# ucsdmanorlab/PSSR2

Hardware: AMD Instinct MI355X
Metric: HR tiles/sec (512^2 4xSR) train (higher is better)
Workload: dtype bf16

## Files before the change

include/pssr_mi355.h:

```cpp
#ifndef PSSR_MI355_H
#define PSSR_MI355_H

#include <stdint.h>

#ifdef __cplusplus
extern "C" {
#endif

typedef void* pssr_stream_t;

enum { PSSR_F32 = 0, PSSR_BF16 = 1, PSSR_F16 = 2 };

enum {
    PSSR_OK = 0,
    PSSR_ERR_ARG = -1,
    PSSR_ERR_LAUNCH = -2,
    PSSR_ERR_UNSUPPORTED = -3
};

int pssr_abi_version(void);
const char* pssr_last_error(void);

int pssr_pack_conv_weight(const float* w_oihw, void* packed, int cout, int cin, int ks,
                          int ci_begin, int ci_count, int mode, const int32_t* n_perm,
// ... 140 lines not shown
int pssr_f64_to_f32(const double* in, float* out, int n, int accumulate, int stripes, pssr_stream_t stream);

int pssr_ssim_level_fwd(const float* x, const float* y, int planes, int h, int w, const float* win_host,
                        int k, float c1, float c2, double* sums, double* l1_sum, pssr_stream_t stream);
int pssr_avgpool2_planes(const float* in, float* out, int planes, int h, int w, pssr_stream_t stream);
int pssr_msssim_weights(const double* sums, int levels, int planes, const double* nvalid,
                        const float* level_weights, int ms, float mix, const double* l1_sum,
                        double l1_numel, const float* grad_out, float* loss_out, float* wts,
                        float* l1_coef, pssr_stream_t stream);
int pssr_ssim_level_bwd(const float* x, const float* y, int planes, int h, int w, const float* win_host,
                        int k, float c1, float c2, const float* wts, int use_ssim, const float* dcoarse,
                        int hc, int wc, const float* l1_coef, float* dx, pssr_stream_t stream);

int pssr_ssim_level_fwd_adj(const float* x, const float* y, float in_div, int planes, int h, int w, const float* win_host, int k,
                            float c1, float c2, int use_ssim, double* sums, double* l1_sum, int stripes, int64_t stripe_stride,
                            float* adj, pssr_stream_t stream);
int pssr_msssim_weights_striped(const double* sums, int stripes, int64_t stripe_stride, double* folded, int levels, int planes,
                                const double* nvalid, const float* level_weights, int ms, float mix, const double* l1_sum,
                                double l1_numel, const float* grad_out, float* loss_out, float* wts, float* l1_coef,
                                pssr_stream_t stream);
int pssr_ssim_level_bwd_adj(const float* x, const float* y, float in_div, const float* adj, int planes, int h, int w,
                            const float* win_host, int k, const float* wts, const float* dcoarse, int hc, int wc,
                            const float* l1_coef, float* dx, pssr_stream_t stream);
int pssr_avgpool2_planes_div(const float* in, float in_div, float* out, int planes, int h, int w, pssr_stream_t stream);
int pssr_avgpool2_pair_div(const float* x, const float* y, float in_div, float* xo, float* yo, int planes, int h, int w,
                           pssr_stream_t stream);

int pssr_adamw_step(float* p, const float* g, float* m, float* v, int64_t n, float lr, float beta1,
                    float beta2, float eps, float weight_decay, int64_t step, float grad_scale,
                    pssr_stream_t stream);
int pssr_adamw_step_dev(float* p, const float* g, float* m, float* v, int64_t n, int64_t* state,
                        float beta1, float beta2, float eps, float weight_decay, float grad_scale,
                        pssr_stream_t stream);
int pssr_amp_check(const float* g, int64_t n, int32_t* amp, pssr_stream_t stream);
int pssr_adamw_step_amp(float* p, const float* g, float* m, float* v, int64_t n, int64_t* state,
                        float beta1, float beta2, float eps, float weight_decay, float grad_scale,
                        int32_t* amp, float growth, float backoff, int interval, pssr_stream_t stream);

int pssr_bilinear_down_u8(const uint8_t* hr, uint8_t* tmp, uint8_t* lr, int planes, int H, int W,
                          int h, int w, pssr_stream_t stream);
int pssr_u8_to_f32(const uint8_t* in, float* out, int64_t n, pssr_stream_t stream);
int pssr_crappify_gaussian(const float* in, float* out, int tiles, int64_t per_tile, float intensity,
                           float gain, float spread, uint64_t seed, uint64_t tile_offset,
                           const double* noise, int flags, const uint64_t* tile_counter,
                           pssr_stream_t stream);
int pssr_crappify_poisson(const float* in, float* out, int tiles, int64_t per_tile, float intensity,
// ... 152 lines not shown
```

pssr2_amd/_lib.py:

```python
from __future__ import annotations

import ctypes as C
import os
from pathlib import Path

_LIB_PATH = Path(__file__).resolve().parent / "libpssr_mi355.so"
_lib = None

F32, BF16, F16 = 0, 1, 2
PRO_NONE, PRO_BN_RELU, PRO_GELU = 0, 1, 2
EPI_STORE, EPI_TAIL, EPI_DGRAD_MASK, EPI_FINAL, EPI_DGRAD_GELU, EPI_HEADQ = 0, 1, 2, 3, 4, 5
FLAG_RELU, FLAG_STATS, FLAG_AFFINE, FLAG_HEADQ, FLAG_SHUF2, FLAG_SOLO = 1, 2, 4, 8, 16, 32

c_void_p, c_int, c_i64, c_float = C.c_void_p, C.c_int, C.c_int64, C.c_float


class ConvDesc(C.Structure):
    _fields_ = [
        ("dtype", C.c_int32), ("n", C.c_int32), ("h", C.c_int32), ("w", C.c_int32),
        ("in0", c_void_p), ("in0_cstride", C.c_int32), ("in0_coff", C.c_int32), ("cin0", C.c_int32), ("taps0", C.c_int32),
        ("w0", c_void_p),
        ("in1", c_void_p), ("in1_cstride", C.c_int32), ("in1_coff", C.c_int32), ("cin1", C.c_int32), ("taps1", C.c_int32),
        ("w1", c_void_p),
        ("prologue", C.c_int32), ("pro_scale", c_void_p), ("pro_shift", c_void_p),
        ("out", c_void_p), ("out_cstride", C.c_int32), ("out_coff", C.c_int32), ("cout", C.c_int32), ("n_pad", C.c_int32),
        ("bias", c_void_p),
        ("epilogue", C.c_int32), ("flags", C.c_int32),
        ("aux", c_void_p), ("aux_cstride", C.c_int32), ("aux_coff", C.c_int32),
        ("aux_scale", c_void_p), ("aux_shift", c_void_p), ("aux_mean", c_void_p), ("aux_invstd", c_void_p),
        ("stats", c_void_p),
# ... 33 lines not shown
    _fields_ = [("w", C.c_void_p * DWPACK_BATCH_MAX), ("packed", C.c_void_p * DWPACK_BATCH_MAX), ("c", C.c_int32 * DWPACK_BATCH_MAX),
                ("flip", C.c_int32 * DWPACK_BATCH_MAX)]


class CopyBatch(C.Structure):
    _fields_ = [("dst", C.c_void_p * COPY_BATCH_MAX), ("src", C.c_void_p * COPY_BATCH_MAX), ("n", C.c_int64 * COPY_BATCH_MAX)]


class PackItem(C.Structure):
    _fields_ = [("w", c_void_p), ("packed", c_void_p), ("n_perm", c_void_p),
                ("cout", C.c_int32), ("cin", C.c_int32), ("ks", C.c_int32), ("ci_begin", C.c_int32), ("ci_count", C.c_int32),
                ("mode", C.c_int32), ("k_pad", C.c_int32), ("n_pad", C.c_int32), ("dtype", C.c_int32), ("center", C.c_int32)]


def lib():
    global _lib
    if _lib is None:
        if not _LIB_PATH.exists():
            raise RuntimeError(
                f"{_LIB_PATH} not found: build the HIP extension first (python -c 'import __graft_entry__ as g; g.build()' "
                "or make -C pssr2_amd/csrc). pssr2_amd has no CPU fallback.")
        import torch
        _lib = C.CDLL(str(_LIB_PATH))
        _lib.pssr_last_error.restype = C.c_char_p
        _lib.pssr_packed_weight_bytes.restype = C.c_int64
        _lib.pssr_conv2d_workspace_bytes.restype = C.c_int64
        _lib.pssr_gradhist_workspace_bytes.restype = C.c_int64
    return _lib


def check(status: int, what: str):
    if status != 0:
        raise RuntimeError(f"{what} failed ({status}): {lib().pssr_last_error().decode()}")


def ptr(t):
    return None if t is None else c_void_p(t.data_ptr())


def stream_ptr():
    import torch
    return c_void_p(torch.cuda.current_stream().cuda_stream)
```

pssr2_amd/csrc/api_common.cpp:

```cpp
#include <stdarg.h>
#include <stdio.h>
#include <stdlib.h>
#include <string.h>

#include <mutex>

#include "tunables.h"

static thread_local char g_err[512] = "";

void pssr_set_error(const char* fmt, ...) {
    va_list ap;
    va_start(ap, fmt);
    vsnprintf(g_err, sizeof(g_err), fmt, ap);
    va_end(ap);
}

extern "C" const char* pssr_last_error(void) { return g_err; }
extern "C" int pssr_abi_version(void) { return 4; }

namespace {
struct Entry { const char* name; int PssrTunables::*field; int dflt; int lo, hi; };
const Entry kEntries[] = {
    {"IGEMM_FLAT", &PssrTunables::igemm_flat, 1, 0, 1},
    {"IGEMM_BIG", &PssrTunables::igemm_big, 1, 0, 2},
    {"IGEMM_V3", &PssrTunables::igemm_v3, 1, 0, 2},
    {"IGEMM_V3_64", &PssrTunables::igemm_v3_64, 1, 0, 1},
    {"V3_LDS_PAD", &PssrTunables::v3_lds_pad, 0, 0, 100},
    {"IGEMM_DBG", &PssrTunables::igemm_dbg, 0, 0, 255},
    {"IGEMM_N64", &PssrTunables::igemm_n64, 1, 0, 1},
    {"IGEMM_KSPLIT", &PssrTunables::igemm_ksplit, 384, 1, 1 << 20},
    {"CONV_EPI8", &PssrTunables::conv_epi8, 1, 0, 1},
    {"WGRAD_LEAN", &PssrTunables::wgrad_lean, 1, 0, 1},
    {"WGRAD_X2", &PssrTunables::wgrad_x2, 0, 0, 1},
    {"WGRAD_DMA", &PssrTunables::wgrad_dma, 1, 0, 1},
    {"WGRAD_BLOCKS", &PssrTunables::wgrad_blocks, 256, 1, 1 << 20},
    {"WGRAD_BLOCKS_1X1", &PssrTunables::wgrad_blocks_1x1, 384, 1, 1 << 20},
    {"DWCONV_TILE", &PssrTunables::dwconv_tile, 1, 0, 1},
    {"DWWG_BLOCKS", &PssrTunables::dwwg_blocks, 1024, 1, 1 << 20},
    {"LN_BWD_BLOCKS", &PssrTunables::ln_bwd_blocks, 256, 1, 1 << 20},
    {"LN_DBG", &PssrTunables::ln_dbg, 0, 0, 3},
};
PssrTunables g_tun;
std::once_flag g_tun_once;
void tun_init() {
    for (const Entry& e : kEntries) {
        char key[64];
        snprintf(key, sizeof(key), "PSSR_%s", e.name);
        const char* v = getenv(key);
        int x = v ? atoi(v) : e.dflt;
        if (x < e.lo || x > e.hi) x = e.dflt;
        g_tun.*(e.field) = x;
    }
}
}

PssrTunables& pssr_tunables() {
    std::call_once(g_tun_once, tun_init);
    return g_tun;
}

extern "C" int pssr_set_option(const char* name, int value) {
    if (name == nullptr) { pssr_set_error("pssr_set_option: null name"); return PSSR_ERR_ARG; }
    PssrTunables& t = pssr_tunables();
// ... 20 lines not shown
```

pssr2_amd/csrc/loss.hip:

```cpp
#include "common.h"

namespace {

constexpr int TS = 32;
constexpr int MAXW = 33;

struct Win { float g[MAXW]; int k; };

template <int K_DUMMY>
__global__ __launch_bounds__(256) void ssim_fwd_kernel(const float* __restrict__ X, const float* __restrict__ Y, int H, int W,
                                                       Win win, float C1, float C2, double* sums ,
                                                       double* l1_sum ) {
    extern __shared__ float lds[];
    const int k = win.k, halo = k - 1, IN = TS + halo;
    float* xs = lds;
    float* ys = xs + IN * IN;
    float* hp = ys + IN * IN;
    const int plane = blockIdx.z;
    const int oy0 = blockIdx.y * TS, ox0 = blockIdx.x * TS;
    const int VH = H - halo, VW = W - halo;
    const float* xp = X + (long)plane * H * W;
    const float* yp = Y + (long)plane * H * W;
    const int tid = threadIdx.x;
    float l1 = 0.f;
// ... 353 lines not shown
            const float cs = (2.f * sxy + C2) / Dcs;
            const float Dl = mx * mx + my * my + C1;
            const float lum = (2.f * mx * my + C1) / Dl;
            cs_acc += cs; ss_acc += lum * cs;
        }
    }
    __shared__ float red[3][256];
    red[0][tid] = cs_acc; red[1][tid] = ss_acc; red[2][tid] = l1;
    __syncthreads();
    for (int o = 128; o > 0; o >>= 1) {
        if (tid < o) { red[0][tid] += red[0][tid + o]; red[1][tid] += red[1][tid + o]; red[2][tid] += red[2][tid + o]; }
        __syncthreads();
    }
    if (tid == 0) {
        atomicAdd(sums + plane * 2, (double)red[0][0]);
        atomicAdd(sums + plane * 2 + 1, (double)red[1][0]);
        if (l1_sum) atomicAdd(l1_sum, (double)red[2][0]);
    }
}

template <int K>
__global__ __launch_bounds__(256) void ssim_fwd_adj_k(const float* __restrict__ X, const float* __restrict__ Y, int H, int W,
                                                      Win win, float C1, float C2, double* sums, double* l1_sum, int stripes, long stripe_stride,
                                                      float* __restrict__ adj, int use_ssim, float in_mul) {
    constexpr int halo = K - 1, IN = TS + halo, SEG = 8, NS = TS / SEG;
    constexpr int HPW = TS + 1;
    extern __shared__ float lds[];
    float* xs = lds;
    float* ys = xs + IN * IN;
    float* hp = ys + IN * IN;
    const int plane = blockIdx.z;
    const int oy0 = blockIdx.y * TS, ox0 = blockIdx.x * TS;
    const int VH = H - halo, VW = W - halo;
    const float* xp = X + (long)plane * H * W;
    const float* yp = Y + (long)plane * H * W;
    const int tid = threadIdx.x;
    float l1 = 0.f;
    for (int i = tid; i < IN * IN; i += 256) {
        const int r = i / IN, c = i % IN;
        const int gy = oy0 + r, gx = ox0 + c;
        float xv = 0.f, yv = 0.f;
        if (gy < H && gx < W) { xv = __fmul_rn(xp[(long)gy * W + gx], in_mul); yv = __fmul_rn(yp[(long)gy * W + gx], in_mul); }
        xs[i] = xv; ys[i] = yv;
    }
    __syncthreads();
    if (l1_sum) {
        constexpr int r5 = K / 2;
        float wsum = 0.f;
#pragma unroll
        for (int t = 0; t < K; ++t) wsum += win.g[t];
        for (int i = tid; i < TS * TS; i += 256) {
            const int r = i / TS, c = i % TS;
            const int gy = oy0 + r, gx = ox0 + c;
            if (gy < H && gx < W) {
                float sy = wsum, sx = wsum;
                if (gy < r5 || gy >= H - r5) {
                    sy = 0.f;
#pragma unroll
                    for (int t = 0; t < K; ++t) { const int yy = gy + t - r5; if (yy >= 0 && yy < H) sy += win.g[t]; }
                }
                if (gx < r5 || gx >= W - r5) {
                    sx = 0.f;
#pragma unroll
                    for (int t = 0; t < K; ++t) { const int xx = gx + t - r5; if (xx >= 0 && xx < W) sx += win.g[t]; }
                }
                l1 += fabsf(xs[r * IN + c] - ys[r * IN + c]) * sy * sx;
            }
        }
// ... 46 lines not shown
            if (use_ssim) {
                const float dl_dmx = 2.f * (my - lum * mx) / Dl;
                a = lum * dcs_dmx + cs * dl_dmx; b = lum * dcs_dexx; cc = lum * dcs_dexy;
            }
            float* ap = adj + ((long)plane * 3 * H + (oy0 + vr0 + j)) * W + ox0 + vc;
            ap[0] = a; ap[(long)H * W] = b; ap[2L * H * W] = cc;
        }
    }
    __shared__ float red[3][256];
    red[0][tid] = cs_acc; red[1][tid] = ss_acc; red[2][tid] = l1;
    __syncthreads();
    for (int o = 128; o > 0; o >>= 1) {
        if (tid < o) { red[0][tid] += red[0][tid + o]; red[1][tid] += red[1][tid + o]; red[2][tid] += red[2][tid + o]; }
        __syncthreads();
    }
    if (tid == 0) {
        const long so = (long)((blockIdx.x + blockIdx.y * 5) % stripes) * stripe_stride, lo = (long)stripes * stripe_stride;
        stat_add(sums + so + plane * 2, lo, red[0][0]);
        stat_add(sums + so + plane * 2 + 1, lo, red[1][0]);
        if (l1_sum) stat_add(l1_sum + so, lo, red[2][0]);
    }
}

template <int K>
__global__ __launch_bounds__(256) void ssim_bwd_adj_k(const float* __restrict__ X, const float* __restrict__ Y, const float* __restrict__ ADJ,
                                                      int H, int W, Win win, const float* __restrict__ wts,
                                                      const float* __restrict__ dcoarse, int HC, int WC, const float* l1_coef_p,
                                                      float* __restrict__ dX, float in_mul) {
    constexpr int halo = K - 1, AD = TS + halo;
    constexpr int SEG = 8, NS = TS / SEG;
    constexpr int ADC = AD + 1;
    constexpr int THR = AD + SEG, THW = TS + 1;
    constexpr int NL = (AD * AD + 255) / 256;
    extern __shared__ float lds[];
    float* ad = lds;
    float* th = lds + AD * ADC;
    const int plane = blockIdx.z;
    const int qy0 = blockIdx.y * TS, qx0 = blockIdx.x * TS;
    const int VH = H - halo, VW = W - halo;
    const float* xp = X + (long)plane * H * W;
    const float* yp = Y + (long)plane * H * W;
    const float* ap = ADJ + (long)plane * 3 * H * W;
    const int tid = threadIdx.x;
    const float wt = wts[plane];
    int goff[NL], lslot[NL];
#pragma unroll
    for (int u = 0; u < NL; ++u) {
        const int i = tid + u * 256;
        const int r = i / AD, c = i - r * AD;
        const int py = qy0 - halo + r, px = qx0 - halo + c;
        lslot[u] = i < AD * AD ? r * ADC + c : -1;
        goff[u] = (i < AD * AD && py >= 0 && py < VH && px >= 0 && px < VW) ? py * W + px : -1;
    }
    float pre[NL];
#define SB_LOAD(Q)                                                                                                \
    _Pragma("unroll") for (int u = 0; u < NL; ++u) pre[u] = goff[u] >= 0 ? wt * ap[(long)(Q) * H * W + goff[u]] : 0.f;
    SB_LOAD(0)
    const bool vitem = tid < TS * NS;
    const int vc = tid % TS, vr0 = (tid / TS) * SEG;
    float xv[SEG], yv[SEG], gsum[SEG];
#pragma unroll
    for (int o = 0; o < SEG; ++o) {
        const int gy = qy0 + vr0 + o, gx = qx0 + vc;
        const bool ok = vitem && gy < H && gx < W;
        xv[o] = ok ? __fmul_rn(xp[(long)gy * W + gx], in_mul) : 0.f;
        yv[o] = ok ? __fmul_rn(yp[(long)gy * W + gx], in_mul) : 0.f;
        gsum[o] = 0.f;
    }
#pragma unroll
    for (int q = 0; q < 3; ++q) {
#pragma unroll
        for (int u = 0; u < NL; ++u) if (lslot[u] >= 0) ad[lslot[u]] = pre[u];
        __syncthreads();
        if (q < 2) { SB_LOAD(q + 1) }
        for (int it = tid; it < AD * NS; it += 256) {
            const int r = it / NS, c0 = (it % NS) * SEG;
            float v[SEG + K - 1];
#pragma unroll
            for (int j = 0; j < SEG + K - 1; ++j) v[j] = ad[r * ADC + c0 + j];
#pragma unroll
            for (int o = 0; o < SEG; ++o) {
                float s_ = 0.f;
#pragma unroll
                for (int t = 0; t < K; ++t) s_ = fmaf(win.g[t], v[o + halo - t], s_);
                th[r * THW + c0 + o] = s_;
            }
        }
        __syncthreads();
        if (vitem) {
            float v[SEG + K - 1];
#pragma unroll
            for (int j = 0; j < SEG + K - 1; ++j) v[j] = th[(vr0 + j) * THW + vc];
#pragma unroll
            for (int o = 0; o < SEG; ++o) {
                float a = 0.f;
#pragma unroll
                for (int t = 0; t < K; ++t) a = fmaf(win.g[t], v[o + halo - t], a);
                if (q == 0) gsum[o] = a;
                else if (q == 1) gsum[o] = gsum[o] + 2.f * xv[o] * a;
                else gsum[o] = gsum[o] + yv[o] * a;
            }
        }
    }
#undef SB_LOAD
    if (!vitem) return;
    const float l1c = l1_coef_p ? l1_coef_p[0] : 0.f;
    constexpr int r5 = K / 2;
    float wsum = 0.f;
#pragma unroll
    for (int t = 0; t < K; ++t) wsum += win.g[t];
    float* dxp = dX + (long)plane * H * W;
#pragma unroll
    for (int o = 0; o < SEG; ++o) {
        const int gy = qy0 + vr0 + o, gx = qx0 + vc;
        if (gy >= H || gx >= W) continue;
        float g = gsum[o];
        if (dcoarse) {
            const int cy = (gy + (H & 1)) >> 1, cx = (gx + (W & 1)) >> 1;
            g += 0.25f * dcoarse[((long)plane * HC + cy) * WC + cx];
        }
        if (l1c != 0.f) {
            float sy = wsum, sx = wsum;
            if (gy < r5 || gy >= H - r5) {
                sy = 0.f;
#pragma unroll
                for (int t = 0; t < K; ++t) { const int yy = gy + t - r5; if (yy >= 0 && yy < H) sy += win.g[t]; }
            }
            if (gx < r5 || gx >= W - r5) {
                sx = 0.f;
#pragma unroll
                for (int t = 0; t < K; ++t) { const int xx = gx + t - r5; if (xx >= 0 && xx < W) sx += win.g[t]; }
            }
            const float d = xv[o] - yv[o];
            g += l1c * sy * sx * (d > 0.f ? 1.f : (d < 0.f ? -1.f : 0.f));
        }
        dxp[(long)gy * W + gx] = __fmul_rn(g, in_mul);
// ... 173 lines not shown
int pssr_ssim_level_fwd(const float* x, const float* y, int planes, int h, int w, const float* win_host, int k,
                        float c1, float c2, double* sums, double* l1_sum, pssr_stream_t s) {
    PSSR_CHECK(x && y && sums && win_host && planes > 0 && k > 0 && k <= MAXW && (k & 1), PSSR_ERR_ARG, "ssim_level_fwd: bad args");
    PSSR_CHECK(h >= k && w >= k, PSSR_ERR_ARG, "ssim_level_fwd: image %dx%d smaller than window %d", h, w, k);
    const int IN = TS + k - 1;
    const size_t lds = (size_t)(2 * IN * IN + 5 * IN * (TS + 1)) * sizeof(float);
    const int eh = l1_sum ? h : h - k + 1, ew = l1_sum ? w : w - k + 1;
    static bool attr = false;
    if (!attr) {
        (void)hipFuncSetAttribute((const void*)ssim_fwd_kernel<0>, hipFuncAttributeMaxDynamicSharedMemorySize, 160 * 1024 - 4096);
        (void)hipFuncSetAttribute((const void*)ssim_fwd_k<11>, hipFuncAttributeMaxDynamicSharedMemorySize, 160 * 1024 - 4096);
        attr = true;
    }
    if (k == 11)
        hipLaunchKernelGGL(ssim_fwd_k<11>, dim3(cdiv(ew, TS), cdiv(eh, TS), planes), dim3(256), lds, (hipStream_t)s, x, y, h, w,
                           make_win(win_host, k), c1, c2, sums, l1_sum);
    else
        hipLaunchKernelGGL(ssim_fwd_kernel<0>, dim3(cdiv(ew, TS), cdiv(eh, TS), planes), dim3(256), lds, (hipStream_t)s, x, y, h, w,
                           make_win(win_host, k), c1, c2, sums, l1_sum);
    PSSR_LAUNCH_CHECK();
    return PSSR_OK;
}

int pssr_ssim_level_fwd_adj(const float* x, const float* y, float in_div, int planes, int h, int w, const float* win_host, int k, float c1,
                            float c2, int use_ssim, double* sums, double* l1_sum, int stripes, int64_t stripe_stride, float* adj,
                            pssr_stream_t s) {
    PSSR_CHECK(x && y && sums && win_host && planes > 0 && adj && k == 11, PSSR_ERR_ARG,
               "ssim_level_fwd_adj: needs the adjoint buffer and the 11-tap window (k=%d)", k);
    PSSR_CHECK(h >= k && w >= k && stripes >= 1 && (stripes == 1 || stripe_stride > 0) && in_div > 0.f, PSSR_ERR_ARG, "ssim_level_fwd_adj: bad size / stripes / in_div");
    const int IN = TS + k - 1;
    const size_t lds = (size_t)(2 * IN * IN + IN * (TS + 1)) * sizeof(float);
    const int eh = l1_sum ? h : h - k + 1, ew = l1_sum ? w : w - k + 1;
    hipLaunchKernelGGL(ssim_fwd_adj_k<11>, dim3(cdiv(ew, TS), cdiv(eh, TS), planes), dim3(256), lds, (hipStream_t)s, x, y, h, w,
                       make_win(win_host, k), c1, c2, sums, l1_sum, stripes, (long)stripe_stride, adj, use_ssim, in_div == 1.f ? 1.f : 1.f / in_div);
    PSSR_LAUNCH_CHECK();
    return PSSR_OK;
}

int pssr_ssim_level_bwd_adj(const float* x, const float* y, float in_div, const float* adj, int planes, int h, int w, const float* win_host,
                            int k, const float* wts, const float* dcoarse, int hc, int wc, const float* l1_coef, float* dx, pssr_stream_t s) {
    PSSR_CHECK(x && y && adj && wts && dx && win_host && planes > 0 && k == 11, PSSR_ERR_ARG, "ssim_level_bwd_adj: bad args (k=%d)", k);
    constexpr int AD = TS + 10;
    const size_t lds = (size_t)(AD * (AD + 1) + (AD + 8) * (TS + 1)) * sizeof(float);
    hipLaunchKernelGGL(ssim_bwd_adj_k<11>, dim3(cdiv(w, TS), cdiv(h, TS), planes), dim3(256), lds, (hipStream_t)s, x, y, adj, h, w,
                       make_win(win_host, k), wts, dcoarse, hc, wc, l1_coef, dx, in_div == 1.f ? 1.f : 1.f / in_div);
    PSSR_LAUNCH_CHECK();
    return PSSR_OK;
}

int pssr_avgpool2_planes(const float* in, float* out, int planes, int h, int w, pssr_stream_t s) {
    return pssr_avgpool2_planes_div(in, 1.f, out, planes, h, w, s);
}

int pssr_avgpool2_planes_div(const float* in, float in_div, float* out, int planes, int h, int w, pssr_stream_t s) {
    PSSR_CHECK(in && out && planes > 0 && h > 0 && w > 0 && in_div > 0.f, PSSR_ERR_ARG, "avgpool2_planes: bad args");
    const int ho = (h + 2 * (h & 1) - 2) / 2 + 1, wo = (w + 2 * (w & 1) - 2) / 2 + 1;
    const long total = (long)planes * ho * wo;
    int blocks = (int)((total + 255) / 256); if (blocks > 8192) blocks = 8192;
    hipLaunchKernelGGL(avgpool_kernel, dim3(blocks), dim3(256), 0, (hipStream_t)s, in, out, in, out, planes, h, w, ho, wo, in_div == 1.f ? 1.f : 1.f / in_div);
    PSSR_LAUNCH_CHECK();
    return PSSR_OK;
}

int pssr_avgpool2_pair_div(const float* x, const float* y, float in_div, float* xo, float* yo, int planes, int h, int w, pssr_stream_t s) {
    PSSR_CHECK(x && y && xo && yo && planes > 0 && h > 0 && w > 0 && in_div > 0.f, PSSR_ERR_ARG, "avgpool2_pair: bad args");
    const int ho = (h + 2 * (h & 1) - 2) / 2 + 1, wo = (w + 2 * (w & 1) - 2) / 2 + 1;
    const long total = (long)planes * ho * wo;
    int blocks = (int)((total + 255) / 256); if (blocks > 8192) blocks = 8192;
    hipLaunchKernelGGL(avgpool_kernel, dim3(blocks, 2), dim3(256), 0, (hipStream_t)s, x, xo, y, yo, planes, h, w, ho, wo, in_div == 1.f ? 1.f : 1.f / in_div);
    PSSR_LAUNCH_CHECK();
// ... 49 lines not shown
```

pssr2_amd/csrc/tunables.h:

```cpp
#pragma once
#include "../../include/pssr_mi355.h"

struct PssrTunables {
    int igemm_flat;
    int igemm_big;
    int igemm_v3;
    int igemm_v3_64;
    int v3_lds_pad;
    int igemm_dbg;
    int igemm_n64;
    int igemm_ksplit;
    int conv_epi8;
    int wgrad_lean;
    int wgrad_x2;
    int wgrad_dma;
    int wgrad_blocks;
    int wgrad_blocks_1x1;
    int dwconv_tile;
    int dwwg_blocks;
    int ln_bwd_blocks;
    int ln_dbg;
};
PssrTunables& pssr_tunables();
```

pssr2_amd/ops.py:

```python
from __future__ import annotations

import ctypes as C

import torch

from . import _lib as L

TORCH_DTYPE = {L.F32: torch.float32, L.BF16: torch.bfloat16, L.F16: torch.float16}


def dtype_code(dt: torch.dtype) -> int:
    if dt == torch.float32:
        return L.F32
    if dt == torch.bfloat16:
        return L.BF16
    if dt == torch.float16:
        return L.F16
    raise ValueError(f"unsupported compute dtype {dt}; use torch.float32, torch.bfloat16 or torch.float16")


def pad_to(v: int, m: int) -> int:
    return (v + m - 1) // m * m


# ... 210 lines not shown

def f64_to_f32_batch(items, stripes=STAT_STRIPES):
    for k in range(0, len(items), L.COPY_BATCH_MAX):
        chunk = items[k:k + L.COPY_BATCH_MAX]
        fb = L.FoldBatch()
        for i, (src, dst, acc) in enumerate(chunk):
            if src.dtype != torch.float64 or dst.dtype != torch.float32 or src.numel() < stripes * dst.numel() or not (src.is_contiguous() and dst.is_contiguous()):
                raise ValueError("f64_to_f32_batch needs contiguous float64 [stripes * n] sources and float32 [n] destinations")
            fb.dst[i], fb.src[i], fb.n[i], fb.accumulate[i] = dst.data_ptr(), src.data_ptr(), dst.numel(), int(acc)
        L.check(L.lib().pssr_f64_to_f32_batch(C.byref(fb), len(chunk), stripes, L.stream_ptr()), "pssr_f64_to_f32_batch")


def _win(win):
    arr = (C.c_float * len(win))(*[float(v) for v in win])
    return arr, len(win)


def ssim_level_fwd(x, y, planes, h, w, win, c1, c2, sums, l1_sum=None):
    arr, k = _win(win)
    L.check(L.lib().pssr_ssim_level_fwd(L.ptr(x), L.ptr(y), planes, h, w, arr, k, C.c_float(c1), C.c_float(c2), L.ptr(sums),
                                        L.ptr(l1_sum), L.stream_ptr()), "pssr_ssim_level_fwd")


def ssim_level_fwd_adj(x, y, planes, h, w, win, c1, c2, use_ssim, sums, l1_sum, stripes, stripe_stride, adj, in_div=1.0):
    k = len(win); arr = (C.c_float * k)(*win)
    L.check(L.lib().pssr_ssim_level_fwd_adj(L.ptr(x), L.ptr(y), C.c_float(in_div), planes, h, w, arr, k, C.c_float(c1), C.c_float(c2), int(use_ssim), L.ptr(sums),
                                            L.ptr(l1_sum), stripes, C.c_int64(stripe_stride), L.ptr(adj), L.stream_ptr()), "pssr_ssim_level_fwd_adj")


def msssim_weights_striped(sums, stripes, stripe_stride, folded, levels, planes, nvalid, level_weights, ms, mix, l1_sum, l1_numel, grad_out,
                           loss_out, wts, l1_coef):
    L.check(L.lib().pssr_msssim_weights_striped(L.ptr(sums), stripes, C.c_int64(stripe_stride), L.ptr(folded), levels, planes, L.ptr(nvalid),
                                                L.ptr(level_weights), int(ms), C.c_float(mix), L.ptr(l1_sum), C.c_double(l1_numel),
                                                L.ptr(grad_out), L.ptr(loss_out), L.ptr(wts), L.ptr(l1_coef), L.stream_ptr()),
            "pssr_msssim_weights_striped")


def ssim_level_bwd_adj(x, y, adj, planes, h, w, win, wts, dcoarse, hc, wc, l1_coef, dx, in_div=1.0):
    k = len(win); arr = (C.c_float * k)(*win)
    L.check(L.lib().pssr_ssim_level_bwd_adj(L.ptr(x), L.ptr(y), C.c_float(in_div), L.ptr(adj), planes, h, w, arr, k, L.ptr(wts), L.ptr(dcoarse), hc, wc,
                                            L.ptr(l1_coef), L.ptr(dx), L.stream_ptr()), "pssr_ssim_level_bwd_adj")


def avgpool2_planes(x, out, planes, h, w, in_div=1.0):
    L.check(L.lib().pssr_avgpool2_planes_div(L.ptr(x), C.c_float(in_div), L.ptr(out), planes, h, w, L.stream_ptr()), "pssr_avgpool2_planes_div")


def avgpool2_pair(x, y, xo, yo, planes, h, w, in_div=1.0):
    L.check(L.lib().pssr_avgpool2_pair_div(L.ptr(x), L.ptr(y), C.c_float(in_div), L.ptr(xo), L.ptr(yo), planes, h, w, L.stream_ptr()),
            "pssr_avgpool2_pair_div")


def msssim_weights(sums, levels, planes, nvalid, level_weights, ms, mix, l1_sum, l1_numel, grad_out, loss_out, wts, l1_coef):
    L.check(L.lib().pssr_msssim_weights(L.ptr(sums), levels, planes, L.ptr(nvalid), L.ptr(level_weights), int(ms), C.c_float(mix),
                                        L.ptr(l1_sum), C.c_double(l1_numel), L.ptr(grad_out), L.ptr(loss_out), L.ptr(wts),
                                        L.ptr(l1_coef), L.stream_ptr()), "pssr_msssim_weights")


def ssim_level_bwd(x, y, planes, h, w, win, c1, c2, wts, use_ssim, dcoarse, hc, wc, l1_coef, dx):
    arr, k = _win(win)
    L.check(L.lib().pssr_ssim_level_bwd(L.ptr(x), L.ptr(y), planes, h, w, arr, k, C.c_float(c1), C.c_float(c2), L.ptr(wts),
                                        int(use_ssim), L.ptr(dcoarse), hc, wc, L.ptr(l1_coef), L.ptr(dx), L.stream_ptr()),
            "pssr_ssim_level_bwd")

# ... 441 lines not shown
```

pssr2_amd/util.py:

```python
from __future__ import annotations

import inspect
import math

import numpy as np
import torch
import torch.nn as nn

from . import ops

MS_WEIGHTS = (0.0448, 0.2856, 0.3001, 0.2363, 0.1333)


def _gauss_1d(size: int, sigma: float):
    coords = torch.arange(size, dtype=torch.float) - size // 2
    g = torch.exp(-(coords ** 2) / (2 * sigma ** 2))
    return (g / g.sum()).tolist()


_CONST_CACHE = {}


class _SSIMLossFunction(torch.autograd.Function):
    @staticmethod
    def forward(ctx, x, y, cfg, in_div=1.0):
        if not x.is_cuda:
            raise RuntimeError("pssr2_amd.SSIMLoss runs on an MI355X (HIP) device only; there is no CPU fallback")
        win, mix, ms, k1, k2, data_range, lvl_w = cfg
        x = x.detach().contiguous().float()
        y = y.detach().contiguous().float()
        n, c, h, w = x.shape
        planes, k = n * c, len(win)
        levels = len(lvl_w) if ms else 1
        if ms and min(h, w) <= (k - 1) * 2 ** 4:
            raise AssertionError(f"Image size should be larger than {(k - 1) * 2 ** 4} due to the 4 downsamplings in ms-ssim")
        c1, c2 = (k1 * data_range) ** 2, (k2 * data_range) ** 2
        dev = x.device
        fused_div = in_div != 1.0 and k == 11 and ctx.needs_input_grad[0]
        if in_div != 1.0 and not fused_div:
            x, y = x / in_div, y / in_div
        div0 = in_div if fused_div else 1.0
        xs, ys, dims = [x], [y], [(h, w)]
        for lv in range(1, levels):
            hh, ww = dims[-1]
            ho, wo = (hh + 2 * (hh & 1) - 2) // 2 + 1, (ww + 2 * (ww & 1) - 2) // 2 + 1
            xo = torch.empty(planes, ho, wo, device=dev)
            yo = torch.empty(planes, ho, wo, device=dev)
            ops.avgpool2_pair(xs[-1], ys[-1], xo, yo, planes, hh, ww, div0 if lv == 1 else 1.0)
            xs.append(xo), ys.append(yo), dims.append((ho, wo))
        adjs = None
        if k == 11 and ctx.needs_input_grad[0]:
            adjs = [torch.empty(planes * 3 * hh * ww, device=dev) for hh, ww in dims]
        stripes = 16 if adjs is not None else 1
        sstride = levels * planes * 2 + 2
        rows = 2 * stripes if stripes > 1 else 1
        sums = torch.zeros(rows * sstride + (sstride if stripes > 1 else 0), dtype=torch.float64, device=dev)
        l1_sum = sums[sstride - 2:sstride - 1] if mix < 1 else None
        for l in range(levels):
            hh, ww = dims[l]
            if adjs is not None:
                ops.ssim_level_fwd_adj(xs[l], ys[l], planes, hh, ww, win, c1, c2, l == levels - 1, sums[l * planes * 2:],
                                       l1_sum if l == 0 else None, stripes, sstride, adjs[l], div0 if l == 0 else 1.0)
            else:
                ops.ssim_level_fwd(xs[l], ys[l], planes, hh, ww, win, c1, c2, sums[l * planes * 2:], l1_sum if l == 0 else None)
        ckey = (tuple(dims), k, tuple(lvl_w) if ms else (1.0,), str(dev))
        cached = _CONST_CACHE.get(ckey)
        if cached is None:
            cached = _CONST_CACHE[ckey] = (
                torch.tensor([float((hh - k + 1) * (ww - k + 1)) for hh, ww in dims], dtype=torch.float64, device=dev),
                torch.tensor(list(lvl_w) if ms else [1.0], dtype=torch.float32, device=dev))
        nvalid, lw = cached
        loss = torch.empty(1, dtype=torch.float32, device=dev)
        wts = torch.empty(levels * planes, dtype=torch.float32, device=dev)
        l1c = torch.empty(1, dtype=torch.float32, device=dev)
        if stripes > 1:
            ops.msssim_weights_striped(sums, stripes, sstride, sums[rows * sstride:], levels, planes, nvalid, lw, ms, mix, l1_sum, float(x.numel()),
                                       None, loss, wts, l1c)
            sums = sums[rows * sstride:]
            l1_sum = sums[levels * planes * 2:levels * planes * 2 + 1] if l1_sum is not None else None
        else:
            ops.msssim_weights(sums, levels, planes, nvalid, lw, ms, mix, l1_sum, float(x.numel()), None, loss, wts, l1c)
        ctx.saved = (xs, ys, dims, sums, nvalid, lw, l1_sum, cfg, planes, x.shape, adjs, div0, in_div if not fused_div else 1.0)
        return loss[0]

    @staticmethod
    def backward(ctx, grad_out):
        xs, ys, dims, sums, nvalid, lw, l1_sum, cfg, planes, shape, adjs, div0, post_div = ctx.saved
        win, mix, ms, k1, k2, data_range, lvl_w = cfg
        levels = len(xs)
        dev = xs[0].device
        c1, c2 = (k1 * data_range) ** 2, (k2 * data_range) ** 2
        go = grad_out.detach().float().reshape(1).contiguous()
        loss = torch.empty(1, dtype=torch.float32, device=dev)
        wts = torch.empty(levels * planes, dtype=torch.float32, device=dev)
        l1c = torch.empty(1, dtype=torch.float32, device=dev)
        ops.msssim_weights(sums, levels, planes, nvalid, lw, ms, mix, l1_sum, float(xs[0].numel()), go, loss, wts, l1c)
        dcoarse, hc, wc = None, 0, 0
        for l in range(levels - 1, -1, -1):
            hh, ww = dims[l]
            dx = torch.empty(planes, hh, ww, device=dev)
            use_ssim = (l == levels - 1)
            l1_arg = l1c if (l == 0 and l1_sum is not None) else None
            if adjs is not None:
                ops.ssim_level_bwd_adj(xs[l], ys[l], adjs[l], planes, hh, ww, win, wts[l * planes:], dcoarse, hc, wc, l1_arg, dx,
                                       div0 if l == 0 else 1.0)
            else:
                ops.ssim_level_bwd(xs[l], ys[l], planes, hh, ww, win, c1, c2, wts[l * planes:], use_ssim, dcoarse, hc, wc, l1_arg, dx)
            dcoarse, hc, wc = dx, hh, ww
        g = dcoarse.view(shape)
        if post_div != 1.0:
            g = g / post_div
        return g, None, None, None


class SSIMLoss(nn.Module):
    def __init__(self, channels: int = 1, mix: float = .8, win_size: int = 11, win_sigma: float = 1.5, ms: bool = True, kwargs=None):
        super().__init__()
        kwargs = {} if kwargs is None else dict(kwargs)
        if win_size % 2 != 1:
            raise ValueError("Window size should be odd.")
        self.K = tuple(kwargs.pop("K", (0.01, 0.03)))
        self.weights = tuple(kwargs.pop("weights", None) or MS_WEIGHTS)
        if kwargs:
            raise TypeError(f"unsupported pytorch_msssim options on the MI355X path: {sorted(kwargs)}")
        self.win = _gauss_1d(win_size, win_sigma)
        self.channels, self.win_size, self.mix, self.ms = channels, win_size, mix, ms

    def forward(self, input, target):
# ... 174 lines not shown
```

Before: 2420.

## Fuse avgpool into SSIM forward, scale grad on load, narrow bwd vertical items

The SSIM forward-adjoint kernel now writes the 2x2-pooled x/y planes for the next level from its LDS tile, which removes the separate avgpool launches and the re-read of the inputs. The backward no longer reruns msssim_weights. It reuses the forward's weights and multiplies by grad_out inside the backward kernel. The backward kernel's vertical pass is templated so each thread handles 4 rows instead of 8 by default, which gives more parallel work per block at the cost of more halo reads. It also adds an ABI version check.

```diff
diff --git a/include/pssr_mi355.h b/include/pssr_mi355.h
--- a/include/pssr_mi355.h
+++ b/include/pssr_mi355.h
@@ -186,6 +186,12 @@
 int pssr_ssim_level_bwd_adj(const float* x, const float* y, float in_div, const float* adj, int planes, int h, int w,
                             const float* win_host, int k, const float* wts, const float* dcoarse, int hc, int wc,
                             const float* l1_coef, float* dx, pssr_stream_t stream);
+int pssr_ssim_level_fwd_adj_pool(const float* x, const float* y, float in_div, int planes, int h, int w, const float* win_host, int k,
+                                 float c1, float c2, int use_ssim, double* sums, double* l1_sum, int stripes, int64_t stripe_stride,
+                                 float* adj, float* pool_x, float* pool_y, pssr_stream_t stream);
+int pssr_ssim_level_bwd_adj_scaled(const float* x, const float* y, float in_div, const float* adj, int planes, int h, int w,
+                                   const float* win_host, int k, const float* wts, const float* dcoarse, int hc, int wc,
+                                   const float* l1_coef, const float* grad_out, float* dx, pssr_stream_t stream);
 int pssr_avgpool2_planes_div(const float* in, float in_div, float* out, int planes, int h, int w, pssr_stream_t stream);
 int pssr_avgpool2_pair_div(const float* x, const float* y, float in_div, float* xo, float* yo, int planes, int h, int w,
                            pssr_stream_t stream);
diff --git a/pssr2_amd/_lib.py b/pssr2_amd/_lib.py
--- a/pssr2_amd/_lib.py
+++ b/pssr2_amd/_lib.py
@@ -6,6 +6,7 @@
 
 _LIB_PATH = Path(__file__).resolve().parent / "libpssr_mi355.so"
 _lib = None
+ABI_VERSION = 5
 
 F32, BF16, F16 = 0, 1, 2
 PRO_NONE, PRO_BN_RELU, PRO_GELU = 0, 1, 2
@@ -85,6 +86,9 @@
                 "or make -C pssr2_amd/csrc). pssr2_amd has no CPU fallback.")
         import torch
         _lib = C.CDLL(str(_LIB_PATH))
+        if _lib.pssr_abi_version() != ABI_VERSION:
+            have, _lib = _lib.pssr_abi_version(), None
+            raise RuntimeError(f"{_LIB_PATH} has ABI version {have}, this package needs {ABI_VERSION}: rebuild it (make -C pssr2_amd/csrc)")
         _lib.pssr_last_error.restype = C.c_char_p
         _lib.pssr_packed_weight_bytes.restype = C.c_int64
         _lib.pssr_conv2d_workspace_bytes.restype = C.c_int64
diff --git a/pssr2_amd/csrc/api_common.cpp b/pssr2_amd/csrc/api_common.cpp
--- a/pssr2_amd/csrc/api_common.cpp
+++ b/pssr2_amd/csrc/api_common.cpp
@@ -17,7 +17,7 @@
 }
 
 extern "C" const char* pssr_last_error(void) { return g_err; }
-extern "C" int pssr_abi_version(void) { return 4; }
+extern "C" int pssr_abi_version(void) { return 5; }
 
 namespace {
 struct Entry { const char* name; int PssrTunables::*field; int dflt; int lo, hi; };
@@ -40,6 +40,7 @@
     {"DWWG_BLOCKS", &PssrTunables::dwwg_blocks, 1024, 1, 1 << 20},
     {"LN_BWD_BLOCKS", &PssrTunables::ln_bwd_blocks, 256, 1, 1 << 20},
     {"LN_DBG", &PssrTunables::ln_dbg, 0, 0, 3},
+    {"SSIM_BWD_WIDE", &PssrTunables::ssim_bwd_wide, 1, 0, 1},
 };
 PssrTunables g_tun;
 std::once_flag g_tun_once;
diff --git a/pssr2_amd/csrc/loss.hip b/pssr2_amd/csrc/loss.hip
--- a/pssr2_amd/csrc/loss.hip
+++ b/pssr2_amd/csrc/loss.hip
@@ -1,4 +1,5 @@
 #include "common.h"
+#include "tunables.h"
 
 namespace {
 
@@ -399,9 +400,11 @@
 template <int K>
 __global__ __launch_bounds__(256) void ssim_fwd_adj_k(const float* __restrict__ X, const float* __restrict__ Y, int H, int W,
                                                       Win win, float C1, float C2, double* sums, double* l1_sum, int stripes, long stripe_stride,
-                                                      float* __restrict__ adj, int use_ssim, float in_mul) {
+                                                      float* __restrict__ adj, int use_ssim, float in_mul,
+                                                      float* __restrict__ pool_x, float* __restrict__ pool_y) {
     constexpr int halo = K - 1, IN = TS + halo, SEG = 8, NS = TS / SEG;
     constexpr int HPW = TS + 1;
+    static_assert((TS / 2) * (TS / 2) == 256, "one pooled pixel per thread");
     extern __shared__ float lds[];
     float* xs = lds;
     float* ys = xs + IN * IN;
@@ -421,6 +424,17 @@
         xs[i] = xv; ys[i] = yv;
     }
     __syncthreads();
+    if (pool_x) {
+        const int pr = tid / (TS / 2), pc = tid % (TS / 2);
+        const int gy = oy0 + 2 * pr, gx = ox0 + 2 * pc;
+        if (gy < H && gx < W) {
+            const int i0 = 2 * pr * IN + 2 * pc;
+            const float sx = __fadd_rn(__fadd_rn(__fadd_rn(__fadd_rn(0.f, xs[i0]), xs[i0 + 1]), xs[i0 + IN]), xs[i0 + IN + 1]);
+            const float sy = __fadd_rn(__fadd_rn(__fadd_rn(__fadd_rn(0.f, ys[i0]), ys[i0 + 1]), ys[i0 + IN]), ys[i0 + IN + 1]);
+            const long po = ((long)plane * (H >> 1) + (gy >> 1)) * (W >> 1) + (gx >> 1);
+            pool_x[po] = __fmul_rn(0.25f, sx); pool_y[po] = __fmul_rn(0.25f, sy);
+        }
+    }
     if (l1_sum) {
         constexpr int r5 = K / 2;
         float wsum = 0.f;
@@ -513,11 +527,11 @@
     }
 }
 
-template <int K>
+template <int K, int VS>
 __global__ __launch_bounds__(256) void ssim_bwd_adj_k(const float* __restrict__ X, const float* __restrict__ Y, const float* __restrict__ ADJ,
                                                       int H, int W, Win win, const float* __restrict__ wts,
                                                       const float* __restrict__ dcoarse, int HC, int WC, const float* l1_coef_p,
-                                                      float* __restrict__ dX, float in_mul) {
+                                                      float* __restrict__ dX, float in_mul, const float* __restrict__ grad_out) {
     constexpr int halo = K - 1, AD = TS + halo;
     constexpr int SEG = 8, NS = TS / SEG;
     constexpr int ADC = AD + 1;
@@ -533,7 +547,8 @@
     const float* yp = Y + (long)plane * H * W;
     const float* ap = ADJ + (long)plane * 3 * H * W;
     const int tid = threadIdx.x;
-    const float wt = wts[plane];
+    const float go = grad_out ? grad_out[0] : 1.f;
+    const float wt = __fmul_rn(wts[plane], go);
     int goff[NL], lslot[NL];
 #pragma unroll
     for (int u = 0; u < NL; ++u) {
@@ -547,11 +562,12 @@
 #define SB_LOAD(Q)                                                                                                \
     _Pragma("unroll") for (int u = 0; u < NL; ++u) pre[u] = goff[u] >= 0 ? wt * ap[(long)(Q) * H * W + goff[u]] : 0.f;
     SB_LOAD(0)
-    const bool vitem = tid < TS * NS;
-    const int vc = tid % TS, vr0 = (tid / TS) * SEG;
-    float xv[SEG], yv[SEG], gsum[SEG];
-#pragma unroll
-    for (int o = 0; o < SEG; ++o) {
+    static_assert(VS == SEG || VS == SEG / 2, "vertical items of SEG or SEG / 2 rows");
+    const bool vitem = tid < TS * (TS / VS);
+    const int vc = tid % TS, vr0 = (tid / TS) * VS;
+    float xv[VS], yv[VS], gsum[VS];
+#pragma unroll
+    for (int o = 0; o < VS; ++o) {
         const int gy = qy0 + vr0 + o, gx = qx0 + vc;
         const bool ok = vitem && gy < H && gx < W;
         xv[o] = ok ? __fmul_rn(xp[(long)gy * W + gx], in_mul) : 0.f;
@@ -579,11 +595,11 @@
         }
         __syncthreads();
         if (vitem) {
-            float v[SEG + K - 1];
-#pragma unroll
-            for (int j = 0; j < SEG + K - 1; ++j) v[j] = th[(vr0 + j) * THW + vc];
-#pragma unroll
-            for (int o = 0; o < SEG; ++o) {
+            float v[VS + K - 1];
+#pragma unroll
+            for (int j = 0; j < VS + K - 1; ++j) v[j] = th[(vr0 + j) * THW + vc];
+#pragma unroll
+            for (int o = 0; o < VS; ++o) {
                 float a = 0.f;
 #pragma unroll
                 for (int t = 0; t < K; ++t) a = fmaf(win.g[t], v[o + halo - t], a);
@@ -595,14 +611,14 @@
     }
 #undef SB_LOAD
     if (!vitem) return;
-    const float l1c = l1_coef_p ? l1_coef_p[0] : 0.f;
+    const float l1c = l1_coef_p ? __fmul_rn(l1_coef_p[0], go) : 0.f;
     constexpr int r5 = K / 2;
     float wsum = 0.f;
 #pragma unroll
     for (int t = 0; t < K; ++t) wsum += win.g[t];
     float* dxp = dX + (long)plane * H * W;
 #pragma unroll
-    for (int o = 0; o < SEG; ++o) {
+    for (int o = 0; o < VS; ++o) {
         const int gy = qy0 + vr0 + o, gx = qx0 + vc;
         if (gy >= H || gx >= W) continue;
         float g = gsum[o];
@@ -822,30 +838,53 @@
     return PSSR_OK;
 }
 
+int pssr_ssim_level_fwd_adj_pool(const float* x, const float* y, float in_div, int planes, int h, int w, const float* win_host, int k, float c1,
+                                 float c2, int use_ssim, double* sums, double* l1_sum, int stripes, int64_t stripe_stride, float* adj,
+                                 float* pool_x, float* pool_y, pssr_stream_t s) {
+    PSSR_CHECK(x && y && sums && win_host && planes > 0 && adj && k == 11, PSSR_ERR_ARG,
+               "ssim_level_fwd_adj: needs the adjoint buffer and the 11-tap window (k=%d)", k);
+    PSSR_CHECK(h >= k && w >= k && stripes >= 1 && (stripes == 1 || stripe_stride > 0) && in_div > 0.f, PSSR_ERR_ARG, "ssim_level_fwd_adj: bad size / stripes / in_div");
+    PSSR_CHECK(!pool_x == !pool_y, PSSR_ERR_ARG, "ssim_level_fwd_adj: the pooled planes come as a pair");
+    PSSR_CHECK(!pool_x || !((h | w) & 1), PSSR_ERR_ARG, "ssim_level_fwd_adj: pooled outputs need even sizes (%dx%d); use pssr_avgpool2_pair_div", h, w);
+    const int IN = TS + k - 1;
+    const size_t lds = (size_t)(2 * IN * IN + IN * (TS + 1)) * sizeof(float);
+    const bool whole = l1_sum || pool_x;
+    const int eh = whole ? h : h - k + 1, ew = whole ? w : w - k + 1;
+    hipLaunchKernelGGL(ssim_fwd_adj_k<11>, dim3(cdiv(ew, TS), cdiv(eh, TS), planes), dim3(256), lds, (hipStream_t)s, x, y, h, w,
+                       make_win(win_host, k), c1, c2, sums, l1_sum, stripes, (long)stripe_stride, adj, use_ssim, in_div == 1.f ? 1.f : 1.f / in_div,
+                       pool_x, pool_y);
+    PSSR_LAUNCH_CHECK();
+    return PSSR_OK;
+}
+
 int pssr_ssim_level_fwd_adj(const float* x, const float* y, float in_div, int planes, int h, int w, const float* win_host, int k, float c1,
                             float c2, int use_ssim, double* sums, double* l1_sum, int stripes, int64_t stripe_stride, float* adj,
                             pssr_stream_t s) {
-    PSSR_CHECK(x && y && sums && win_host && planes > 0 && adj && k == 11, PSSR_ERR_ARG,
-               "ssim_level_fwd_adj: needs the adjoint buffer and the 11-tap window (k=%d)", k);
-    PSSR_CHECK(h >= k && w >= k && stripes >= 1 && (stripes == 1 || stripe_stride > 0) && in_div > 0.f, PSSR_ERR_ARG, "ssim_level_fwd_adj: bad size / stripes / in_div");
-    const int IN = TS + k - 1;
-    const size_t lds = (size_t)(2 * IN * IN + IN * (TS + 1)) * sizeof(float);
-    const int eh = l1_sum ? h : h - k + 1, ew = l1_sum ? w : w - k + 1;
-    hipLaunchKernelGGL(ssim_fwd_adj_k<11>, dim3(cdiv(ew, TS), cdiv(eh, TS), planes), dim3(256), lds, (hipStream_t)s, x, y, h, w,
-                       make_win(win_host, k), c1, c2, sums, l1_sum, stripes, (long)stripe_stride, adj, use_ssim, in_div == 1.f ? 1.f : 1.f / in_div);
-    PSSR_LAUNCH_CHECK();
-    return PSSR_OK;
-}
-
-int pssr_ssim_level_bwd_adj(const float* x, const float* y, float in_div, const float* adj, int planes, int h, int w, const float* win_host,
-                            int k, const float* wts, const float* dcoarse, int hc, int wc, const float* l1_coef, float* dx, pssr_stream_t s) {
+    return pssr_ssim_level_fwd_adj_pool(x, y, in_div, planes, h, w, win_host, k, c1, c2, use_ssim, sums, l1_sum, stripes, stripe_stride, adj,
+                                        nullptr, nullptr, s);
+}
+
+int pssr_ssim_level_bwd_adj_scaled(const float* x, const float* y, float in_div, const float* adj, int planes, int h, int w, const float* win_host,
+                                   int k, const float* wts, const float* dcoarse, int hc, int wc, const float* l1_coef, const float* grad_out,
+                                   float* dx, pssr_stream_t s) {
     PSSR_CHECK(x && y && adj && wts && dx && win_host && planes > 0 && k == 11, PSSR_ERR_ARG, "ssim_level_bwd_adj: bad args (k=%d)", k);
     constexpr int AD = TS + 10;
     const size_t lds = (size_t)(AD * (AD + 1) + (AD + 8) * (TS + 1)) * sizeof(float);
-    hipLaunchKernelGGL(ssim_bwd_adj_k<11>, dim3(cdiv(w, TS), cdiv(h, TS), planes), dim3(256), lds, (hipStream_t)s, x, y, adj, h, w,
-                       make_win(win_host, k), wts, dcoarse, hc, wc, l1_coef, dx, in_div == 1.f ? 1.f : 1.f / in_div);
+    const dim3 grid(cdiv(w, TS), cdiv(h, TS), planes);
+    const float in_mul = in_div == 1.f ? 1.f : 1.f / in_div;
+    if (pssr_tunables().ssim_bwd_wide)
+        hipLaunchKernelGGL((ssim_bwd_adj_k<11, 4>), grid, dim3(256), lds, (hipStream_t)s, x, y, adj, h, w, make_win(win_host, k), wts, dcoarse, hc, wc,
+                           l1_coef, dx, in_mul, grad_out);
+    else
+        hipLaunchKernelGGL((ssim_bwd_adj_k<11, 8>), grid, dim3(256), lds, (hipStream_t)s, x, y, adj, h, w, make_win(win_host, k), wts, dcoarse, hc, wc,
+                           l1_coef, dx, in_mul, grad_out);
     PSSR_LAUNCH_CHECK();
     return PSSR_OK;
+}
+
+int pssr_ssim_level_bwd_adj(const float* x, const float* y, float in_div, const float* adj, int planes, int h, int w, const float* win_host,
+                            int k, const float* wts, const float* dcoarse, int hc, int wc, const float* l1_coef, float* dx, pssr_stream_t s) {
+    return pssr_ssim_level_bwd_adj_scaled(x, y, in_div, adj, planes, h, w, win_host, k, wts, dcoarse, hc, wc, l1_coef, nullptr, dx, s);
 }
 
 int pssr_avgpool2_planes(const float* in, float* out, int planes, int h, int w, pssr_stream_t s) {
diff --git a/pssr2_amd/csrc/tunables.h b/pssr2_amd/csrc/tunables.h
--- a/pssr2_amd/csrc/tunables.h
+++ b/pssr2_amd/csrc/tunables.h
@@ -20,5 +20,6 @@
     int dwwg_blocks;
     int ln_bwd_blocks;
     int ln_dbg;
+    int ssim_bwd_wide;
 };
 PssrTunables& pssr_tunables();
diff --git a/pssr2_amd/ops.py b/pssr2_amd/ops.py
--- a/pssr2_amd/ops.py
+++ b/pssr2_amd/ops.py
@@ -256,10 +256,11 @@
                                         L.ptr(l1_sum), L.stream_ptr()), "pssr_ssim_level_fwd")
 
 
-def ssim_level_fwd_adj(x, y, planes, h, w, win, c1, c2, use_ssim, sums, l1_sum, stripes, stripe_stride, adj, in_div=1.0):
+def ssim_level_fwd_adj(x, y, planes, h, w, win, c1, c2, use_ssim, sums, l1_sum, stripes, stripe_stride, adj, in_div=1.0, pool_x=None, pool_y=None):
     k = len(win); arr = (C.c_float * k)(*win)
-    L.check(L.lib().pssr_ssim_level_fwd_adj(L.ptr(x), L.ptr(y), C.c_float(in_div), planes, h, w, arr, k, C.c_float(c1), C.c_float(c2), int(use_ssim), L.ptr(sums),
-                                            L.ptr(l1_sum), stripes, C.c_int64(stripe_stride), L.ptr(adj), L.stream_ptr()), "pssr_ssim_level_fwd_adj")
+    L.check(L.lib().pssr_ssim_level_fwd_adj_pool(L.ptr(x), L.ptr(y), C.c_float(in_div), planes, h, w, arr, k, C.c_float(c1), C.c_float(c2), int(use_ssim),
+                                                 L.ptr(sums), L.ptr(l1_sum), stripes, C.c_int64(stripe_stride), L.ptr(adj), L.ptr(pool_x), L.ptr(pool_y),
+                                                 L.stream_ptr()), "pssr_ssim_level_fwd_adj_pool")
 
 
 def msssim_weights_striped(sums, stripes, stripe_stride, folded, levels, planes, nvalid, level_weights, ms, mix, l1_sum, l1_numel, grad_out,
@@ -270,10 +271,10 @@
             "pssr_msssim_weights_striped")
 
 
-def ssim_level_bwd_adj(x, y, adj, planes, h, w, win, wts, dcoarse, hc, wc, l1_coef, dx, in_div=1.0):
+def ssim_level_bwd_adj(x, y, adj, planes, h, w, win, wts, dcoarse, hc, wc, l1_coef, dx, in_div=1.0, grad_out=None):
     k = len(win); arr = (C.c_float * k)(*win)
-    L.check(L.lib().pssr_ssim_level_bwd_adj(L.ptr(x), L.ptr(y), C.c_float(in_div), L.ptr(adj), planes, h, w, arr, k, L.ptr(wts), L.ptr(dcoarse), hc, wc,
-                                            L.ptr(l1_coef), L.ptr(dx), L.stream_ptr()), "pssr_ssim_level_bwd_adj")
+    L.check(L.lib().pssr_ssim_level_bwd_adj_scaled(L.ptr(x), L.ptr(y), C.c_float(in_div), L.ptr(adj), planes, h, w, arr, k, L.ptr(wts), L.ptr(dcoarse), hc, wc,
+                                                   L.ptr(l1_coef), L.ptr(grad_out), L.ptr(dx), L.stream_ptr()), "pssr_ssim_level_bwd_adj_scaled")
 
 
 def avgpool2_planes(x, out, planes, h, w, in_div=1.0):
diff --git a/pssr2_amd/util.py b/pssr2_amd/util.py
--- a/pssr2_amd/util.py
+++ b/pssr2_amd/util.py
@@ -2,6 +2,7 @@
 
 import inspect
 import math
+import os
 
 import numpy as np
 import torch
@@ -19,6 +20,8 @@
 
 
 _CONST_CACHE = {}
+
+_LOSS_FUSE = os.environ.get("PSSR_LOSS_FUSE", "1") != "0"
 
 
 class _SSIMLossFunction(torch.autograd.Function):
@@ -40,14 +43,10 @@
         if in_div != 1.0 and not fused_div:
             x, y = x / in_div, y / in_div
         div0 = in_div if fused_div else 1.0
-        xs, ys, dims = [x], [y], [(h, w)]
+        dims = [(h, w)]
         for lv in range(1, levels):
             hh, ww = dims[-1]
-            ho, wo = (hh + 2 * (hh & 1) - 2) // 2 + 1, (ww + 2 * (ww & 1) - 2) // 2 + 1
-            xo = torch.empty(planes, ho, wo, device=dev)
-            yo = torch.empty(planes, ho, wo, device=dev)
-            ops.avgpool2_pair(xs[-1], ys[-1], xo, yo, planes, hh, ww, div0 if lv == 1 else 1.0)
-            xs.append(xo), ys.append(yo), dims.append((ho, wo))
+            dims.append(((hh + 2 * (hh & 1) - 2) // 2 + 1, (ww + 2 * (ww & 1) - 2) // 2 + 1))
         adjs = None
         if k == 11 and ctx.needs_input_grad[0]:
             adjs = [torch.empty(planes * 3 * hh * ww, device=dev) for hh, ww in dims]
@@ -56,11 +55,21 @@
         rows = 2 * stripes if stripes > 1 else 1
         sums = torch.zeros(rows * sstride + (sstride if stripes > 1 else 0), dtype=torch.float64, device=dev)
         l1_sum = sums[sstride - 2:sstride - 1] if mix < 1 else None
+        xs, ys = [x], [y]
         for l in range(levels):
             hh, ww = dims[l]
+            xo = yo = None
+            if l + 1 < levels:
+                xo = torch.empty(planes, *dims[l + 1], device=dev)
+                yo = torch.empty(planes, *dims[l + 1], device=dev)
+                xs.append(xo), ys.append(yo)
+            pool_fused = xo is not None and adjs is not None and _LOSS_FUSE and hh % 2 == 0 and ww % 2 == 0
+            if xo is not None and not pool_fused:
+                ops.avgpool2_pair(xs[l], ys[l], xo, yo, planes, hh, ww, div0 if l == 0 else 1.0)
             if adjs is not None:
                 ops.ssim_level_fwd_adj(xs[l], ys[l], planes, hh, ww, win, c1, c2, l == levels - 1, sums[l * planes * 2:],
-                                       l1_sum if l == 0 else None, stripes, sstride, adjs[l], div0 if l == 0 else 1.0)
+                                       l1_sum if l == 0 else None, stripes, sstride, adjs[l], div0 if l == 0 else 1.0,
+                                       xo if pool_fused else None, yo if pool_fused else None)
             else:
                 ops.ssim_level_fwd(xs[l], ys[l], planes, hh, ww, win, c1, c2, sums[l * planes * 2:], l1_sum if l == 0 else None)
         ckey = (tuple(dims), k, tuple(lvl_w) if ms else (1.0,), str(dev))
@@ -80,21 +89,23 @@
             l1_sum = sums[levels * planes * 2:levels * planes * 2 + 1] if l1_sum is not None else None
         else:
             ops.msssim_weights(sums, levels, planes, nvalid, lw, ms, mix, l1_sum, float(x.numel()), None, loss, wts, l1c)
-        ctx.saved = (xs, ys, dims, sums, nvalid, lw, l1_sum, cfg, planes, x.shape, adjs, div0, in_div if not fused_div else 1.0)
+        ctx.saved = (xs, ys, dims, sums, nvalid, lw, l1_sum, cfg, planes, x.shape, adjs, div0, in_div if not fused_div else 1.0, wts, l1c)
         return loss[0]
 
     @staticmethod
     def backward(ctx, grad_out):
-        xs, ys, dims, sums, nvalid, lw, l1_sum, cfg, planes, shape, adjs, div0, post_div = ctx.saved
+        xs, ys, dims, sums, nvalid, lw, l1_sum, cfg, planes, shape, adjs, div0, post_div, wts, l1c = ctx.saved
         win, mix, ms, k1, k2, data_range, lvl_w = cfg
         levels = len(xs)
         dev = xs[0].device
         c1, c2 = (k1 * data_range) ** 2, (k2 * data_range) ** 2
         go = grad_out.detach().float().reshape(1).contiguous()
-        loss = torch.empty(1, dtype=torch.float32, device=dev)
-        wts = torch.empty(levels * planes, dtype=torch.float32, device=dev)
-        l1c = torch.empty(1, dtype=torch.float32, device=dev)
-        ops.msssim_weights(sums, levels, planes, nvalid, lw, ms, mix, l1_sum, float(xs[0].numel()), go, loss, wts, l1c)
+        go_on_load = adjs is not None and _LOSS_FUSE
+        if not go_on_load:
+            loss = torch.empty(1, dtype=torch.float32, device=dev)
+            wts = torch.empty(levels * planes, dtype=torch.float32, device=dev)
+            l1c = torch.empty(1, dtype=torch.float32, device=dev)
+            ops.msssim_weights(sums, levels, planes, nvalid, lw, ms, mix, l1_sum, float(xs[0].numel()), go, loss, wts, l1c)
         dcoarse, hc, wc = None, 0, 0
         for l in range(levels - 1, -1, -1):
             hh, ww = dims[l]
@@ -103,7 +114,7 @@
             l1_arg = l1c if (l == 0 and l1_sum is not None) else None
             if adjs is not None:
                 ops.ssim_level_bwd_adj(xs[l], ys[l], adjs[l], planes, hh, ww, win, wts[l * planes:], dcoarse, hc, wc, l1_arg, dx,
-                                       div0 if l == 0 else 1.0)
+                                       div0 if l == 0 else 1.0, go if go_on_load else None)
             else:
                 ops.ssim_level_bwd(xs[l], ys[l], planes, hh, ww, win, c1, c2, wts[l * planes:], use_ssim, dcoarse, hc, wc, l1_arg, dx)
             dcoarse, hc, wc = dx, hh, ww
```

Result: no change. 2404 (median of 2 runs) (-0.7%).
